# Emieeel/auto_oo

Hardware: AMD Instinct MI355X
Metric: OO-VQE energy+grad evals/sec (formaldimine CAS(4e,3o)/cc-pVDZ); 2e-transform fp64 TFLOP/s vs roofline (higher is better)
Workload: dtype f64; 1 GPU; configs[1] shape: N=43 AOs, n_occ=6, CAS(4e,3o), UCCD n_theta=4, n_kappa=327; one step = one batched call evaluating energy + full gradient of all 256 geometries of the rank (256 synthetic geometries in the job, geometry g on rank g mod n_gpus); value = evaluations/s; in-order calls on one stream; geometries_per_rank=256, batched_calls=1332, calls=in order, parallelism=geometry-sharded x1, one all_gather at the end, dist_world_size=1, devices_visible=1, device_of_rank0=0

## Files before the change

auto_oo_amd/csrc/cas.hip:

```cpp
#include "plan.h"
#include "circuit_small.h"
#include <type_traits>
#include <stdlib.h>

namespace {

constexpr int HALF_WAVES = 8;
constexpr int TRI_REG_R = 3;
constexpr int tiles_depth(int zt) { return zt == 3 ? 4 : 8; }
constexpr int stream_depth(int zt) { return zt == 3 ? 2 : 3; }
constexpr int AUX_PLAIN = 0, AUX_NT = 2;

constexpr int SYM_FULL = 0, SYM_MIRROR = 1, SYM_PACKED = 2;
__device__ __forceinline__ void tri_decode(long t, int N, int& p, int& q)
{
    const double b = 2.0 * N + 1.0;
    int pp = (int)((b - sqrt(b * b - 8.0 * (double)t)) * 0.5);
    pp = pp < 0 ? 0 : (pp > N - 1 ? N - 1 : pp);
    while (pp > 0 && (long)pp * (2 * N - pp + 1) / 2 > t) --pp;
    while (pp < N - 1 && (long)(pp + 1) * (2 * N - pp) / 2 <= t) ++pp;
    p = pp;
    q = pp + (int)(t - (long)pp * (2 * N - pp + 1) / 2);
}

// ... 2241 lines not shown
    double* d1 = lds;
    double* d2 = d1 + (size_t)M * no;
    double* o1 = d2 + (size_t)M * no;
    double* o2 = o1 + (size_t)no * na2;
    double* cube = o2 + (size_t)no * na2;
    double* FIn = cube + na3;
    double* red = FIn + 64;
    for (int idx = tid; idx < M * no; idx += FROW_THREADS) {
        const int x = idx / no, i = idx - x * no;
        d1[idx] = gn[x * M2 + i * M + i];
        d2[idx] = gn[i * M2 + i * M + x];
    }
    for (int idx = tid; idx < no * na2; idx += FROW_THREADS) {
        const int m = idx / na2, vw = idx - m * na2, v = vw / na, w = vw - v * na;
        o1[idx] = gn[m * M2 + (no + v) * M + no + w];
        o2[idx] = gn[(no + w) * M2 + (no + v) * M + m];
    }
    for (int idx = tid; idx < na3; idx += FROW_THREADS) {
        int t = idx;
        const int y = t % na; t /= na;
        const int x = t % na; t /= na;
        cube[idx] = gn[(no + t) * M2 + (no + x) * M + no + y];
    }
    __syncthreads();
    for (int x = tid; x < M; x += FROW_THREADS) {
        double fi = hmo[(size_t)n * M + x];
        for (int i = 0; i < no; ++i) fi += 2.0 * d1[x * no + i] - d2[x * no + i];
        FIn[x] = fi;
    }
    __syncthreads();
    for (int m = tid; m < M; m += FROW_THREADS) {
        double val;
        if (m < no) {
            double fa = 0.0;
            for (int vw = 0; vw < na2; ++vw) fa += gam[vw] * (o1[m * na2 + vw] - 0.5 * o2[m * na2 + vw]);
            val = 2.0 * ((k == 0 ? FIn[m] : 0.0) + fa);
        } else {
            const int v = m - no;
            const double* Gv = Gam + (size_t)v * na3;
            double acc = 0.0;
            for (int w = 0; w < na; ++w) acc += FIn[no + w] * gam[v * na + w];
            for (int idx = 0; idx < na3; ++idx) acc += Gv[idx] * cube[idx];
            val = acc;
        }
        Fcol[((size_t)k * M + m) * N + n] = val;
    }
    double part = 0.0;
    if (n >= no && n < M) {
        const int p = n - no;
        const double* gp = gam + (size_t)p * na;
        const double* Gp = Gam + (size_t)p * na3;
        for (int q = tid; q < na; q += FROW_THREADS) part += FIn[no + q] * gp[q];
        for (int idx = tid; idx < na3; idx += FROW_THREADS) part += 0.5 * cube[idx] * Gp[idx];
    }
    for (int o = 32; o > 0; o >>= 1) part += __shfl_xor(part, o);
    if ((tid & 63) == 0) red[tid >> 6] = part;
    __syncthreads();
    if (tid == 0) Epart[(size_t)k * N + n] = (red[0] + red[1]) + (red[2] + red[3]);
    if (k == 0) {
        if (tid == 0) Cpart[n] = n < no ? hmo[(size_t)n * M + n] + FIn[n] : 0.0;
        if (n >= no && n < M) {
            const int p = n - no;
            for (int q = tid; q < na; q += FROW_THREADS) c1[p * na + q] = FIn[no + q];
            for (int idx = tid; idx < na3; idx += FROW_THREADS) c2[(size_t)p * na3 + idx] = 0.5 * cube[idx];
        }
    }
}

__global__ __launch_bounds__(512)
void cas_final_kernel(const double* __restrict__ Fcol, const double* __restrict__ Epart,
                      const double* __restrict__ Cpart, double nuc, int nrdm, int N, int M,
                      const int32_t* __restrict__ kap_row, const int32_t* __restrict__ kap_col,
                      int n_kappa, double* __restrict__ c0, double* __restrict__ E,
                      double* __restrict__ gvec, double* __restrict__ dE, double* __restrict__ fock,
                      double* __restrict__ gmat, const double* __restrict__ nuc_arr,
                      size_t out_stride)
{
    const int tid = threadIdx.x;
    {
        const size_t gi = blockIdx.x;
        Fcol += gi * (size_t)nrdm * M * N;
        Epart += gi * (size_t)nrdm * N;
        Cpart += gi * (size_t)N;
        c0 += gi * out_stride;
        E += gi * out_stride;
        gvec += gi * out_stride;
        if (dE) dE += gi * out_stride;
        if (fock) fock += gi * (size_t)N * N;
        if (gmat) gmat += gi * (size_t)N * N;
        if (nuc_arr) nuc = nuc_arr[gi];
    }
    for (long base = 0; base < (long)nrdm * n_kappa; base += 4 * 512) {
        int rr[4], cc[4], kk[4];
#pragma unroll
        for (int u = 0; u < 4; ++u) {
            const long idx = base + u * 512 + tid;
            const bool ok = idx < (long)nrdm * n_kappa;
            const long ii = ok ? idx : 0;
            kk[u] = (int)(ii / n_kappa);
            const int t = (int)(ii - (long)kk[u] * n_kappa);
            rr[u] = kap_row[t];
            cc[u] = kap_col[t];
        }
        double frc[4], fcr[4];
#pragma unroll
        for (int u = 0; u < 4; ++u) {
            const double* F = Fcol + (size_t)kk[u] * M * N;
            const int r = rr[u], c = cc[u];
            frc[u] = F[(size_t)(r < M ? r : 0) * N + c] * (r < M ? 1.0 : 0.0);
            fcr[u] = F[(size_t)(c < M ? c : 0) * N + r] * (c < M ? 1.0 : 0.0);
        }
#pragma unroll
        for (int u = 0; u < 4; ++u) {
            const long idx = base + u * 512 + tid;
            if (idx < (long)nrdm * n_kappa) gvec[idx] = 2.0 * (frc[u] - fcr[u]);
        }
    }
    if (fock)
        for (int idx = tid; idx < N * N; idx += 512) {
            const int m = idx / N;
            fock[idx] = m < M ? Fcol[idx] : 0.0;
        }
    if (gmat)
        for (int idx = tid; idx < N * N; idx += 512) {
            const int m = idx / N, n = idx - m * N;
            const double fmn = m < M ? Fcol[(size_t)m * N + n] : 0.0;
            const double fnm = n < M ? Fcol[(size_t)n * N + m] : 0.0;
            gmat[idx] = 2.0 * (fmn - fnm);
        }
    if (tid < nrdm) {
        const int k = tid;
        double acc = 0.0;
        for (int n = 0; n < M; ++n) acc += Epart[(size_t)k * N + n];
        if (k == 0) {
            double core = nuc;
            for (int n = 0; n < M; ++n) core += Cpart[n];
            c0[0] = core;
            E[0] = core + acc;
        } else if (dE) {
            dE[k - 1] = acc;
        }
    }
}

constexpr int TAIL_THREADS = 512;

__host__ __device__ inline bool tail_needed(int x, int y, int z, int no)
{
    const int lo = y < z ? y : z, hi = y < z ? z : y;
    if (lo >= no) return true;
    if (hi < no) return lo == hi || x == lo || x == hi;
    return x >= no || x == lo;
}

#ifdef OOVQE_TAIL_PROBE
constexpr int TAIL_PROBE_WGS = 512, TAIL_PROBE_MARKS = 32;
__device__ long long g_tail_probe[TAIL_PROBE_WGS][TAIL_PROBE_MARKS];
#define TAIL_MARK(i)                                                                              \
    do {                                                                                          \
        __syncthreads();                                                                          \
        if (threadIdx.x == 0 && blockIdx.x < TAIL_PROBE_WGS && (i) < TAIL_PROBE_MARKS)            \
            g_tail_probe[blockIdx.x][i] = wall_clock64();                                         \
    } while (0)
#else
#define TAIL_MARK(i) do {} while (0)
#endif

template <int KS>
__global__ __launch_bounds__(TAIL_THREADS, 2)
void cas_tail_kernel(const double* __restrict__ J, const double* __restrict__ C, const double* __restrict__ Wpre,
                     const double* __restrict__ gamma, const double* __restrict__ Gamma, int nrdm, int N, int no,
                     int na, int NC, double nuc, const double* __restrict__ nuc_arr,
                     const int32_t* __restrict__ kap_row, const int32_t* __restrict__ kap_col, int n_kappa,
                     double* __restrict__ c0, double* __restrict__ E, double* __restrict__ gvec,
                     double* __restrict__ dE, double* __restrict__ c1, double* __restrict__ c2, size_t out_stride)
{
    extern __shared__ double lds[];
    constexpr int NW = TAIL_THREADS / 64;
    constexpr int PW = (4 * KS + NW - 1) / NW;
    constexpr int GR = 2, NG = (PW + GR - 1) / GR;
    constexpr int NTN = (4 * KS + 15) / 16;
    const int M = no + na, M2 = M * M, M3 = M2 * M;
    const int na2 = na * na, na3 = na2 * na, na4 = na2 * na2;
    const int ncol = M * (M + 1) / 2, nty = (ncol + 15) / 16;
    const long tri = (long)N * (N + 1) / 2;
    const int by = blockIdx.x;
    const int tid = threadIdx.x, lane = tid & 63;
    const int wave = __builtin_amdgcn_readfirstlane(tid >> 6);
    const int lq = lane >> 4, lr = lane & 15;
    {
        const size_t gi = by;
        J += gi * nty * tri * 16;
        C += gi * (size_t)N * N;
        Wpre += gi * (size_t)N * N;
        gamma += gi * (size_t)nrdm * na2;
        Gamma += gi * (size_t)nrdm * na4;
        c0 += gi * out_stride;
        E += gi * out_stride;
        gvec += gi * out_stride;
        if (dE) dE += gi * out_stride;
        c1 += gi * out_stride;
        c2 += gi * out_stride;
        if (nuc_arr) nuc = nuc_arr[gi];
    }
    double* Gc = lds;
    double* Cl = Gc + (size_t)N * NC;
    double* hn = Cl + (size_t)N * M;
    double* FIn = hn + (size_t)N * M;
    double* gml = FIn + (size_t)N * M;
    double* Gml = gml + (size_t)nrdm * na2;
    double* Cp = Gml + (size_t)nrdm * na4;
    int* tab = reinterpret_cast<int*>(Cp + N);
    int* wcnt = tab + M3;
    int* krow = wcnt + NW;
    int* kcol = krow + n_kappa;
    double* scr = Cp + N + (M3 + NW + 2 * n_kappa + 1) / 2;
    const int LDP = M * 16 + 8;

    typedef unsigned v2u __attribute__((ext_vector_type(2)));
    const __amdgpu_buffer_rsrc_t csrd = __builtin_amdgcn_make_buffer_rsrc(
        const_cast<double*>(C), 0, (int)((size_t)N * N * sizeof(double)), 0x00020000);
    double cfa[NTN][KS];
#pragma unroll
    for (int nt = 0; nt < NTN; ++nt)
#pragma unroll
        for (int ks = 0; ks < KS; ++ks) {
            const int pp = 4 * ks + lq, n = 16 * nt + lr;
            const v2u v = __builtin_amdgcn_raw_buffer_load_b64(
                csrd, (pp < N && n < N) ? (unsigned)((pp * N + n) * (int)sizeof(double)) : 0x7fffffffu, 0, 0);
            cfa[nt][ks] = __builtin_bit_cast(double, v);
        }
    constexpr bool COLQ_REGS = KS < 12;
    int colq[KS];
#pragma unroll
    for (int ks = 0; ks < KS; ++ks) {
        const int q = 4 * ks + lq < N ? 4 * ks + lq : N - 1;
        colq[ks] = ((q * (2 * N - q + 1) / 2 - q) * 16 + lr) * (int)sizeof(double);
    }
    const int lin0 = (lq * 16 + lr) * (int)sizeof(double);
    auto load_group = [&](double (&bf)[GR][KS], int ty, int g) {
#pragma unroll
        for (int r = 0; r < GR; ++r) {
            const int i = g * GR + r;
            if (i >= PW) continue;
            int wv = wave;
#if defined(__HIP_DEVICE_COMPILE__)
            asm volatile("" : "+s"(wv));
#endif
            const int p = wv + NW * i;
            int lqo = lq;
#if defined(__HIP_DEVICE_COMPILE__)
            asm volatile("" : "+v"(lqo));
#endif
            const __amdgpu_buffer_rsrc_t jsrd = __builtin_amdgcn_make_buffer_rsrc(
                const_cast<double*>(J + (size_t)(ty < nty ? ty : 0) * tri * 16), 0,
                p < N && ty < nty ? (int)(tri * 16 * sizeof(double)) : 0, 0x00020000);
            const int colp = p * 16 * (int)sizeof(double);
            const int rowp = (p * (2 * N - p + 1) / 2 - p) * 16 * (int)sizeof(double) + lin0;
#pragma unroll
            for (int ks = 0; ks < KS; ++ks) {
                const int q = 4 * ks + lqo;
                const int cq = COLQ_REGS ? colq[ks] : (q * (2 * N - 1 - q) / 2 * 16 + lr) * (int)sizeof(double);
                const int off = lq < p - 4 * ks ? cq + colp : rowp + ks * 64 * (int)sizeof(double);
                const v2u v = __builtin_amdgcn_raw_buffer_load_b64(jsrd, (unsigned)off, 0, 0);
                bf[r][ks] = __builtin_bit_cast(double, v);
            }
        }
    };
    double* T3s = scr;
    auto mfma_group = [&](const double (&af)[KS], const double (&bf)[GR][KS], int g) {
#pragma unroll
        for (int r = 0; r < GR; ++r) {
            const int i = g * GR + r;
            if (i >= PW) continue;
            int wv = wave;
#if defined(__HIP_DEVICE_COMPILE__)
            asm volatile("" : "+s"(wv));
#endif
            const int p = wv + NW * i;
            if (p >= 4 * KS) continue;
            d4 acc = d4{0.0, 0.0, 0.0, 0.0};
            if (p < N) {
#pragma unroll
                for (int ks = 0; ks < KS; ++ks) acc = mfma_f64(af[ks], bf[r][ks], acc);
            }
            double* row = T3s + (p * LDP + lq * 16 + lr);
#pragma unroll
            for (int j = 0; j < 4; ++j)
                if (lq + 4 * j < M) row[j * 64] = acc[j];
        }
    };
    double bs[2][GR][KS];
    TAIL_MARK(0);
#pragma unroll
    for (int s0 = 0; s0 < 2; ++s0) load_group(bs[s0], s0 / NG, s0 % NG);

    for (int idx = tid; idx < N * M; idx += TAIL_THREADS) {
        const int q = idx / M, x = idx - q * M;
        Cl[idx] = C[(size_t)q * N + x];
    }
    for (int idx = tid; idx < N * N; idx += TAIL_THREADS) scr[idx] = Wpre[idx];
    for (int idx = tid; idx < nrdm * na2; idx += TAIL_THREADS) gml[idx] = gamma[idx];
    for (int idx = tid; idx < nrdm * na4; idx += TAIL_THREADS) Gml[idx] = Gamma[idx];
    for (int idx = tid; idx < n_kappa; idx += TAIL_THREADS) {
        krow[idx] = kap_row[idx];
        kcol[idx] = kap_col[idx];
    }
    TAIL_MARK(1);
    {
        const int total = M * ncol;
        int base = 0;
        for (int i0 = 0; i0 < total; i0 += TAIL_THREADS) {
            const int i = i0 + tid;
            int x = 0, y = 0, z = 0;
            bool need = false;
            if (i < total) {
                x = i / ncol;
                tri_decode(i - x * ncol, M, y, z);
                need = tail_needed(x, y, z, no);
            }
            const unsigned long long mask = __ballot(need);
            const int below = __popcll(mask & ((1ull << lane) - 1ull));
            if (lane == 0) wcnt[wave] = __popcll(mask);
            __syncthreads();
            int pre = base, all = 0;
            for (int w = 0; w < NW; ++w) {
                const int c = wcnt[w];
                if (w < wave) pre += c;
                all += c;
            }
            if (i < total) {
                const int v = need ? pre + below : -1;
                tab[(x * M + y) * M + z] = v;
                tab[(x * M + z) * M + y] = v;
            }
            __syncthreads();
            base += all;
        }
    }
    TAIL_MARK(2);
    for (int idx = tid; idx < N * M; idx += TAIL_THREADS) {
        const int n = idx / M, x = idx - n * M;
        double acc = 0.0;
        for (int q = 0; q < N; ++q) acc += scr[(size_t)n * N + q] * Cl[q * M + x];
        hn[idx] = acc;
    }
    __syncthreads();
    TAIL_MARK(3);

    {
        const int ntn = (N + 15) / 16;
        auto tail_tile = [&](auto par, int ty) {
            constexpr int P = decltype(par)::value;
            double af[KS];
            int lqv = lq;
#if defined(__HIP_DEVICE_COMPILE__)
            asm volatile("" : "+v"(lqv));
#endif
#pragma unroll
            for (int ks = 0; ks < KS; ++ks) {
                const int q = 4 * ks + lqv;
                const double c = Cl[(q < N ? q : N - 1) * M + (lr < M ? lr : 0)];
                af[ks] = (q < N && lr < M) ? c : 0.0;
            }
#pragma unroll
            for (int g = 0; g < NG; ++g) {
                mfma_group(af, bs[(P + g) & 1], g);
                __builtin_amdgcn_sched_barrier(0);
                load_group(bs[(P + g) & 1], ty + (g + 2) / NG, (g + 2) % NG);
                __builtin_amdgcn_sched_barrier(0);
                if (g == 0) TAIL_MARK(ty < 3 ? 4 + 3 * ty : 31);
            }
            __syncthreads();
            TAIL_MARK(ty < 3 ? 5 + 3 * ty : 31);
            const int yz = 16 * ty + lr;
            int off = 0;
            if (yz < ncol) {
                int y, z;
                tri_decode(yz, M, y, z);
                off = y * M + z;
            }
#pragma unroll
            for (int nt = 0; nt < NTN; ++nt) {
                if (nt >= ntn) continue;
                const int t0 = nt * M;
                for (int tile = t0 + (wave - t0 % NW + NW) % NW; tile < t0 + M; tile += NW) {
                    const int x = tile - t0;
                    double tf[KS];
#pragma unroll
                    for (int ks = 0; ks < KS; ++ks) tf[ks] = T3s[(size_t)(4 * ks + lq) * LDP + x * 16 + lr];
                    d4 acc = d4{0.0, 0.0, 0.0, 0.0};
#pragma unroll
                    for (int ks = 0; ks < KS; ++ks) acc = mfma_f64(cfa[nt][ks], tf[ks], acc);
                    const int ci = yz < ncol ? tab[x * M2 + off] : -1;
                    if (ci >= 0) {
#pragma unroll
                        for (int j = 0; j < 4; ++j) {
                            const int n = 16 * nt + lq + 4 * j;
                            if (n < N) Gc[(size_t)n * NC + ci] = acc[j];
                        }
                    }
                }
            }
            __syncthreads();
            TAIL_MARK(ty < 3 ? 6 + 3 * ty : 31);
        };
        for (int ty = 0; ty < nty; ty += 2) {
            tail_tile(std::integral_constant<int, 0>{}, ty);
            if (ty + 1 < nty) tail_tile(std::integral_constant<int, NG & 1>{}, ty + 1);
        }
    }

#define TAIL_G(n, a, b, c) Gc[(size_t)(n) * NC + tab[((a) * M + (b)) * M + (c)]]
    for (int idx = tid; idx < N * M; idx += TAIL_THREADS) {
        const int n = idx / M, x = idx - n * M;
        double fi = hn[idx];
        for (int i = 0; i < no; ++i) fi += 2.0 * TAIL_G(n, x, i, i) - TAIL_G(n, i, i, x);
        FIn[idx] = fi;
    }
    TAIL_MARK(13);
    double* Fl = scr;
    double* El = Fl + (size_t)nrdm * M * N;
    double* Ga = El + (size_t)nrdm * N;
    double* Dc = Ga + (size_t)N * na3;
    for (int idx = tid; idx < N * na3; idx += TAIL_THREADS) {
        const int n = idx / na3, r = idx - n * na3;
        const int w = r / na2, x = (r / na) % na, y = r % na;
        Ga[idx] = TAIL_G(n, no + w, no + x, no + y);
    }
    for (int idx = tid; idx < N * no * na2; idx += TAIL_THREADS) {
        const int n = idx / (no * na2), r = idx - n * (no * na2);
        const int m = r / na2, v = (r / na) % na, w = r % na;
        const int V = no + v, W = no + w;
        Dc[idx] = TAIL_G(n, m, V, W) - 0.5 * TAIL_G(n, W, V, m);
    }
    __syncthreads();
    TAIL_MARK(14);
    for (int n = tid; n < N; n += TAIL_THREADS) Cp[n] = n < no ? hn[n * M + n] + FIn[n * M + n] : 0.0;
    for (int idx = tid; idx < na * (na + na3); idx += TAIL_THREADS) {
        const int pl = idx / (na + na3), r0 = idx - pl * (na + na3);
        const int n = no + pl;
        if (r0 < na) {
            c1[pl * na + r0] = FIn[n * M + no + r0];
        } else {
            int t = r0 - na;
            const int i3 = t;
            const int s = t % na; t /= na;
            const int r = t % na; t /= na;
            const int q = t;
            c2[(size_t)pl * na3 + i3] = 0.5 * TAIL_G(n, no + q, no + r, no + s);
        }
    }
    TAIL_MARK(15);
    const int ncore = N * nrdm * no;
    for (int idx = tid; idx < N * nrdm * M; idx += TAIL_THREADS) {
        int n, k, m;
        if (idx < ncore) {
            n = idx / (nrdm * no);
            const int r0 = idx - n * (nrdm * no);
            k = r0 / no;
            m = r0 - k * no;
        } else {
            const int j = idx - ncore;
            n = j / (nrdm * na);
            const int r0 = j - n * (nrdm * na);
            k = r0 / na;
            m = no + r0 - k * na;
        }
        const double* FIv = FIn + (size_t)n * M;
        const double* gam = gml + (size_t)k * na2;
        double val;
        if (m < no) {
            const double* Dm = Dc + ((size_t)n * no + m) * na2;
            double fa = 0.0;
            for (int v = 0; v < na; ++v)
                for (int w = 0; w < na; ++w) fa += gam[v * na + w] * Dm[v * na + w];
            val = 2.0 * ((k == 0 ? FIv[m] : 0.0) + fa);
        } else {
            const int v = m - no;
            const double* Gv = Gml + (size_t)k * na4 + (size_t)v * na3;
            double acc = 0.0;
            for (int w = 0; w < na; ++w) acc += FIv[no + w] * gam[v * na + w];
            for (int w = 0; w < na; ++w)
                for (int x = 0; x < na; ++x)
                    for (int y = 0; y < na; ++y)
                        acc += Gv[(w * na + x) * na + y] * Ga[(size_t)n * na3 + (w * na + x) * na + y];
            val = acc;
        }
        Fl[((size_t)k * M + m) * N + n] = val;
    }
    TAIL_MARK(16);
    for (int idx = tid; idx < N * nrdm; idx += TAIL_THREADS) {
        const int n = idx / nrdm, k = idx - n * nrdm;
        double acc = 0.0;
        if (n >= no && n < M) {
            const int p = n - no;
            const double* FIv = FIn + (size_t)n * M;
            const double* gam = gml + (size_t)k * na2 + (size_t)p * na;
            const double* Gpq = Gml + (size_t)k * na4 + (size_t)p * na3;
            for (int q = 0; q < na; ++q) acc += FIv[no + q] * gam[q];
            for (int q = 0; q < na; ++q)
                for (int r = 0; r < na; ++r)
                    for (int s2 = 0; s2 < na; ++s2)
                        acc += 0.5 * Ga[(size_t)n * na3 + (q * na + r) * na + s2] * Gpq[(q * na + r) * na + s2];
        }
        El[(size_t)k * N + n] = acc;
    }
#undef TAIL_G
    __syncthreads();
    TAIL_MARK(17);

    for (int idx = tid; idx < nrdm * n_kappa; idx += TAIL_THREADS) {
        const int k = idx / n_kappa, t = idx - k * n_kappa;
        const int r = krow[t], c = kcol[t];
        const double* F = Fl + (size_t)k * M * N;
        const double frc = F[(size_t)(r < M ? r : 0) * N + c] * (r < M ? 1.0 : 0.0);
        const double fcr = F[(size_t)(c < M ? c : 0) * N + r] * (c < M ? 1.0 : 0.0);
        gvec[idx] = 2.0 * (frc - fcr);
    }
    if (tid < nrdm) {
        const int k = tid;
        double acc = 0.0;
        for (int n = 0; n < M; ++n) acc += El[(size_t)k * N + n];
        if (k == 0) {
            double core = nuc;
            for (int n = 0; n < M; ++n) core += Cp[n];
            c0[0] = core;
            E[0] = core + acc;
        } else if (dE) {
            dE[k - 1] = acc;
        }
    }
    TAIL_MARK(18);
}

}

#ifdef OOVQE_TAIL_PROBE
extern "C" int oovqe_tail_probe_read(long long* out, int n)
{
    const size_t bytes = sizeof(long long) * (size_t)(n < TAIL_PROBE_WGS * TAIL_PROBE_MARKS ? n : TAIL_PROBE_WGS * TAIL_PROBE_MARKS);
    return hipMemcpyFromSymbol(out, HIP_SYMBOL(g_tail_probe), bytes) == hipSuccess ? 0 : 1;
}
#endif

#define OOVQE_STAGE1_DISPATCH(v, LAUNCH, ...)                                                     \
    switch ((v).kch) {                                                                            \
    case 4: LAUNCH(4, 1, 2, ##__VA_ARGS__); break;                                                \
    case 8: LAUNCH(8, 2, 5, ##__VA_ARGS__); break;                                                \
    case 11: LAUNCH(11, 3, 8, ##__VA_ARGS__); break;                                              \
    default: LAUNCH(12, 3, 10, ##__VA_ARGS__); break;                                             \
    }
#define OOVQE_KS_DISPATCH(v, LAUNCH)                                                              \
    switch ((v).ks) {                                                                             \
    case 4: LAUNCH(4); break;                                                                     \
    case 8: LAUNCH(8); break;                                                                     \
    default: LAUNCH(12); break;                                                                   \
    }

static int stage1_variant(int N, Stage1Variant* v)
{
    static const Stage1Variant rows[] = {{4, 1, 2, 4}, {8, 2, 5, 8}, {11, 3, 8, 12}, {12, 3, 10, 12}};
    for (const Stage1Variant& r : rows)
        if (N >= 1 && (N + 3) / 4 <= r.kch) {
            *v = r;
            return 0;
        }
    oovqe_set_error("cas_eval: no stage-1 kernel variant for N=%d", N);
    return OOVQE_ERR_ARG;
}

static size_t half_lds_bytes(int N, int M)
{
    const int ZT = (M + 15) / 16, nrb = (N + 15) / 16, LDM = 16 * (ZT | 1);
    return (((size_t)nrb * 16 * LDM + 511) / 512) * 512 * sizeof(double);
}
static size_t half_lds_bytes_rs(int N, int M) { return half_lds_bytes(N, M) + (size_t)HALF_WAVES * 16 * 17 * sizeof(double); }

static int stage1_half(int N, int M, int sym, bool rs, bool tiles, Stage1* s)
{
    memset(s, 0, sizeof(*s));
    OOVQE_REQUIRE(N >= 1 && M >= 1 && M <= N, "cas_half_transform: bad N=%d M=%d", N, M);
    const int ZT = (M + 15) / 16, nrb = (N + 15) / 16, ksteps = (N + 3) / 4;
    OOVQE_REQUIRE(ZT <= 3, "cas_half_transform: n_occ+ncas = %d > 48 not supported", M);
    OOVQE_REQUIRE(half_lds_bytes(N, M) <= 160 * 1024, "cas_half_transform: N=%d M=%d needs %zu B of LDS", N, M,
                  half_lds_bytes(N, M));
    s->zt = ZT;
    s->sym = sym;
    if (nrb <= 3) {
        s->kernel = S1_HALF;
        if (int rc = stage1_variant(N, &s->v)) return rc;
        snprintf(s->name, sizeof(s->name), "half_transform_kernel<%d,%d,%d>%s", ZT, s->v.kch, s->v.nrb,
                 sym ? " (slabs p <= q)" : "");
        return 0;
    }
    int waste = 1 << 30;
    for (int k = 16; k >= 10; --k) {
        const int w = (ksteps + k - 1) / k * k - ksteps;
        if (w < waste) { waste = w; s->skch = k; }
    }
    s->rs = rs && half_lds_bytes_rs(N, M) <= 160 * 1024;
    if (tiles && s->rs && sym == SYM_MIRROR) {
        s->kernel = S1_TILES;
        snprintf(s->name, sizeof(s->name), "half_tiles_kernel<%d,%d>", ZT, tiles_depth(ZT));
    } else {
        s->kernel = S1_STREAM;
        snprintf(s->name, sizeof(s->name), "half_stream_kernel<%d,%d,%d,%s>", ZT, s->skch, stream_depth(ZT), s->rs ? "true" : "false");
    }
    return 0;
}

static int half_transform_batched(const double* g_ao, const double* C, int N, int M, double* T2, int batch,
                                  oovqe_stream_t stream, const Stage1& s, double* Vk_tri = nullptr,
                                  const double* g_tiles = nullptr)
{
    OOVQE_REQUIRE(g_ao && C && T2, "cas_half_transform: null pointer");
    OOVQE_REQUIRE(!Vk_tri || (s.sym == SYM_MIRROR && N <= 48),
                  "cas_half_transform: the quarter-transformed output needs p<->q symmetric integrals and N <= 48");
    OOVQE_REQUIRE(batch >= 1 && batch <= 65535, "cas_half_transform: batch=%d", batch);
    OOVQE_REQUIRE(s.kernel != S1_TILES || g_tiles, "cas_half_transform: no tile-packed integrals");
    hipStream_t st = (hipStream_t)stream;
    const int ZT = s.zt, sym = s.sym;
    const int nrb = (N + 15) / 16;
    const long nslabs = sym == SYM_FULL ? (long)N * N : (long)N * (N + 1) / 2;
    const long want = (nslabs + HALF_WAVES - 1) / HALF_WAVES;
    oovqe_note_stage1("%s", s.name);
    oovqe_profile_mark_start(st);
    if (s.kernel == S1_HALF) {
#define OOVQE_LAUNCH_HALF(KC_, NS_, NPC_, Z)                                                      \
    do {                                                                                          \
        const unsigned wpg = 4u;                                                \
        hipLaunchKernelGGL((half_transform_kernel<Z, KC_, NS_>),                                  \
                           dim3((unsigned)((nslabs + wpg - 1) / wpg), batch), dim3(wpg * 64),     \
                           0, st, g_ao, C, T2, N, M, nslabs, sym, Vk_tri);                        \
    } while (0)
        if (ZT == 1) OOVQE_STAGE1_DISPATCH(s.v, OOVQE_LAUNCH_HALF, 1)
        else if (ZT == 2) OOVQE_STAGE1_DISPATCH(s.v, OOVQE_LAUNCH_HALF, 2)
        else OOVQE_STAGE1_DISPATCH(s.v, OOVQE_LAUNCH_HALF, 3)
#undef OOVQE_LAUNCH_HALF
    } else if (s.kernel == S1_TILES) {
        const long slab_doubles = (long)nrb * (nrb + 1) / 2 * 256;
        const size_t lds_rs = half_lds_bytes_rs(N, M);
#define OOVQE_LAUNCH_TILES(Z, D_, A_)                                                             \
    do {                                                                                          \
        const void* fn = (const void*)half_tiles_kernel<Z, D_, A_>;                               \
        int rc_ = oovqe_ensure_dynamic_lds(fn, 160 * 1024);                                       \
        if (rc_) return rc_;                                                                      \
        long per = (long)oovqe_cu_count() / batch;               \
        if (per < 1) per = 1;                                                                     \
        if (per > want) per = want;                                                               \
        hipLaunchKernelGGL((half_tiles_kernel<Z, D_, A_>), dim3((unsigned)per, batch),            \
                           dim3(HALF_WAVES * 64), lds_rs, st, g_tiles, C, T2, N, M, nrb, nslabs,  \
                           nslabs * slab_doubles);                                                \
    } while (0)
        if (ZT == 1) OOVQE_LAUNCH_TILES(1, tiles_depth(1), AUX_NT);
        else if (ZT == 3) OOVQE_LAUNCH_TILES(3, tiles_depth(3), AUX_NT);
        else OOVQE_LAUNCH_TILES(2, tiles_depth(2), AUX_NT);
#undef OOVQE_LAUNCH_TILES
    } else {
        const int snkc = ((N + 3) / 4 + s.skch - 1) / s.skch;
#define OOVQE_LAUNCH_STREAM(Z, KC_, D_)                                                           \
    do {                                                                                          \
        if (s.rs) OOVQE_LAUNCH_STREAM_RS(Z, KC_, D_, true, half_lds_bytes_rs(N, M));              \
        else OOVQE_LAUNCH_STREAM_RS(Z, KC_, D_, false, half_lds_bytes(N, M));                     \
    } while (0)
#define OOVQE_LAUNCH_STREAM_RS(Z, KC_, D_, RS_, lds_bytes_)                                       \
    do {                                                                                          \
        const void* fn = (const void*)half_stream_kernel<Z, KC_, D_, RS_>;                        \
        const size_t lds_bytes = lds_bytes_;                                                      \
        if (int rc_ = oovqe_ensure_dynamic_lds(fn, 160 * 1024)) return rc_;                       \
        const int occ = oovqe_blocks_per_cu(fn, HALF_WAVES * 64, lds_bytes);                      \
        if (occ < 0) return occ;                                                                  \
        long per = ((long)occ * oovqe_cu_count()) / batch;                                        \
        if (per < 1) per = 1;                                                                     \
        if (per > want) per = want;                                                               \
        hipLaunchKernelGGL((half_stream_kernel<Z, KC_, D_, RS_>), dim3((unsigned)per, batch),     \
                           dim3(HALF_WAVES * 64), lds_bytes, st, g_ao, C, T2, N, M, nrb, snkc,    \
                           nslabs, sym);                                                          \
    } while (0)
#define OOVQE_DISPATCH_STREAM(Z, D_)                                                              \
    do {                                                                                          \
        switch (s.skch) {                                                                         \
        case 10: OOVQE_LAUNCH_STREAM(Z, 10, D_); break;                                           \
        case 11: OOVQE_LAUNCH_STREAM(Z, 11, D_); break;                                           \
        case 12: OOVQE_LAUNCH_STREAM(Z, 12, D_); break;                                           \
        case 13: OOVQE_LAUNCH_STREAM(Z, 13, D_); break;                                           \
// ... 4 lines not shown
    } while (0)
        if (ZT == 1) OOVQE_DISPATCH_STREAM(1, stream_depth(1));
        else if (ZT == 2) OOVQE_DISPATCH_STREAM(2, stream_depth(2));
        else OOVQE_DISPATCH_STREAM(3, stream_depth(3));
#undef OOVQE_DISPATCH_STREAM
#undef OOVQE_LAUNCH_STREAM
#undef OOVQE_LAUNCH_STREAM_RS
    }
    oovqe_profile_mark_stop(st);
    OOVQE_CHECK_LAUNCH(s.kernel == S1_TILES ? "cas_half_transform/tiles" : "cas_half_transform");
    return 0;
}

extern "C" int oovqe_cas_half_transform(const double* g_ao, const double* C, int N, int M, double* T2,
                                        oovqe_stream_t stream)
{
    Stage1 s;
    if (int rc = stage1_half(N, M, SYM_FULL, false, false, &s)) return rc;
    return half_transform_batched(g_ao, C, N, M, T2, 1, stream, s);
}

extern "C" int oovqe_eri_symmetry_flags(const double* g_ao, int N, int batch, unsigned* eri_flags,
                                        oovqe_stream_t stream)
{
    OOVQE_REQUIRE(g_ao && eri_flags, "eri_symmetry_flags: null pointer");
    OOVQE_REQUIRE(N >= 1 && N <= 65535 && batch >= 1 && batch <= 65535, "eri_symmetry_flags: N=%d batch=%d",
                  N, batch);
    hipStream_t st = (hipStream_t)stream;
    int* flag = nullptr;
    OOVQE_CHECK_HIP(hipMalloc(&flag, sizeof(int)), "eri_symmetry_flags");
    hipError_t e = hipMemsetAsync(flag, 0, sizeof(int), st);
    if (e == hipSuccess) {
        hipLaunchKernelGGL(eri_symmetry_check_kernel, dim3(N, N, batch), dim3(256), 0, st,
                           reinterpret_cast<const unsigned long long*>(g_ao), N, flag);
        e = hipGetLastError();
    }
    int bad = 3;
    if (e == hipSuccess) e = hipMemcpyAsync(&bad, flag, sizeof(int), hipMemcpyDeviceToHost, st);
    if (e == hipSuccess) e = hipStreamSynchronize(st);
    (void)hipFree(flag);
    OOVQE_CHECK_HIP(e, "eri_symmetry_flags");
    *eri_flags = ((bad & 1) ? 0u : OOVQE_ERI_PQ_SYMMETRIC) | ((bad & 2) ? 0u : OOVQE_ERI_RS_SYMMETRIC);
    return 0;
}

extern "C" int oovqe_eri_ingest(const double* g_ao, int N, int batch, double* packed, unsigned* eri_flags,
                                oovqe_stream_t stream)
{
    OOVQE_REQUIRE(g_ao && eri_flags, "eri_ingest: null pointer");
    OOVQE_REQUIRE(N >= 1 && N <= 4096 && batch >= 1 && batch <= 65535, "eri_ingest: N=%d batch=%d", N, batch);
    hipStream_t st = (hipStream_t)stream;
    if (N > 48) {
        for (int gi = 0; gi < batch; ++gi) {
            int rc = oovqe_eri_symmetry_flags(g_ao + (size_t)gi * N * N * N * N, N, 1, eri_flags + gi, stream);
            if (rc) return rc;
        }
        return packed ? oovqe_eri_pack(g_ao, N, batch, packed, stream) : 0;
    }
    int* flag = nullptr;
    OOVQE_CHECK_HIP(hipMalloc(&flag, sizeof(int) * (size_t)batch), "eri_ingest");
    hipError_t e = hipMemsetAsync(flag, 0, sizeof(int) * (size_t)batch, st);
    if (e == hipSuccess) {
        hipLaunchKernelGGL(eri_ingest_kernel, dim3((unsigned)(N * (N + 1) / 2), batch), dim3(256), 0, st,
                           reinterpret_cast<const unsigned long long*>(g_ao), packed, N, eri_slab_pitch(N), flag);
        e = hipGetLastError();
    }
    int* bad = (int*)malloc(sizeof(int) * (size_t)batch);
    if (!bad) e = hipErrorOutOfMemory;
    if (e == hipSuccess) e = hipMemcpyAsync(bad, flag, sizeof(int) * (size_t)batch, hipMemcpyDeviceToHost, st);
    if (e == hipSuccess) e = hipStreamSynchronize(st);
    (void)hipFree(flag);
    if (e == hipSuccess)
        for (int gi = 0; gi < batch; ++gi)
            eri_flags[gi] = ((bad[gi] & 1) ? 0u : OOVQE_ERI_PQ_SYMMETRIC) | ((bad[gi] & 2) ? 0u : OOVQE_ERI_RS_SYMMETRIC);
    free(bad);
    OOVQE_CHECK_HIP(e, "eri_ingest");
    return 0;
}

static int sym_q_contract_batched(const double* J, const double* C, double* T3, int N, int M, int batch,
                                  hipStream_t st)
{
    OOVQE_REQUIRE(M >= 1 && M <= 16 && N >= 1 && N <= 48, "sym_q_contract: N=%d M=%d", N, M);
    Stage1Variant v;
    if (int rc = stage1_variant(N, &v)) return rc;
    const unsigned threads = (unsigned)((M * M + 15) / 16 * 64);
    oovqe_profile_mark_start_l(st, LABEL_Q_TO_X);
#define OOVQE_LAUNCH_Q(KS_) \
    hipLaunchKernelGGL(sym_q_contract_kernel<KS_>, dim3(N, batch), dim3(threads), 0, st, J, C, T3, N, M)
    OOVQE_KS_DISPATCH(v, OOVQE_LAUNCH_Q)
#undef OOVQE_LAUNCH_Q
    oovqe_profile_mark_stop(st);
    OOVQE_CHECK_LAUNCH("cas_eval/sym_q_contract");
    return 0;
}

static int sym_gm_batched(const double* J, const double* C, double* Gm, int N, int M, int batch,
                          hipStream_t st, const oovqe_circuit_job_t* cj, bool packed)
{
    OOVQE_REQUIRE(M >= 1 && M <= 16 && N >= 1 && N <= 48, "sym_gm: N=%d M=%d", N, M);
    Stage1Variant v;
    if (int rc = stage1_variant(N, &v)) return rc;
    size_t lds_bytes = (size_t)4 * v.ks * (M * 16 + 8) * sizeof(double);
    if (cj && cj->lds_bytes > lds_bytes) lds_bytes = cj->lds_bytes;
    const unsigned nty = (unsigned)(((packed ? M * (M + 1) / 2 : M * M) + 15) / 16);
    oovqe_circuit_job_t job;
    memset(&job, 0, sizeof(job));
    if (cj) job = *cj;
    const unsigned nx = nty + (cj ? 1 : 0);
    const bool xcd_grid = batch > 1 && oovqe_opt(OOVQE_OPT_GM_PLAIN_GRID) == 0;
    const dim3 grid = xcd_grid ? dim3(nx * (unsigned)((batch + 7) / 8 * 8)) : dim3(nx, batch);
#define OOVQE_LAUNCH_GM2(KS_, WPE_)                                                               \
    do {                                                                                          \
        if (int rc_ = oovqe_ensure_dynamic_lds((const void*)sym_gm_kernel<KS_, WPE_>, lds_bytes)) return rc_; \
        hipLaunchKernelGGL((sym_gm_kernel<KS_, WPE_>), grid, dim3(SMALL_THREADS), lds_bytes, st,  \
                           J, C, Gm, N, M, packed ? 1 : 0, job, cj ? 1 : 0, batch);               \
    } while (0)
    const bool multi_round = ((long)nx * batch > (long)oovqe_cu_count() || oovqe_opt(OOVQE_OPT_GM_TWO_PER_CU)) &&
                             2 * lds_bytes <= 160 * 1024 && oovqe_opt(OOVQE_OPT_GM_ONE_PER_CU) == 0;
#define OOVQE_LAUNCH_GM(KS_)                                                                      \
    do {                                                                                          \
        if (multi_round) OOVQE_LAUNCH_GM2(KS_, 4);                                                \
        else OOVQE_LAUNCH_GM2(KS_, 2);                                                            \
    } while (0)
    oovqe_profile_mark_start_l(st, LABEL_P_TO_N);
    OOVQE_KS_DISPATCH(v, OOVQE_LAUNCH_GM)
    oovqe_profile_mark_stop(st);
#undef OOVQE_LAUNCH_GM
#undef OOVQE_LAUNCH_GM2
    OOVQE_CHECK_LAUNCH("cas_eval/sym_gm");
    return 0;
}

static int tail_depth(int N, const Stage1Variant& v) { return N >= 41 && N <= 44 ? 11 : v.ks; }
#define OOVQE_TAIL_DISPATCH(ks, LAUNCH)                                                           \
    switch (ks) {                                                                                 \
    case 4: LAUNCH(4); break;                                                                     \
    case 8: LAUNCH(8); break;                                                                     \
    case 11: LAUNCH(11); break;                                                                   \
    default: LAUNCH(12); break;                                                                   \
    }

static size_t tail_lds_bytes(int N, int no, int na, int nrdm, int n_kappa, int* NC)
{
    const int M = no + na, M3 = M * M * M;
    Stage1Variant v;
    if (N > 48 || M > 16 || stage1_variant(N, &v)) return 0;
    int nc = 0;
    for (int x = 0; x < M; ++x)
        for (int y = 0; y < M; ++y)
            for (int z = y; z < M; ++z) nc += tail_needed(x, y, z, no) ? 1 : 0;
    *NC = nc;
    const size_t na2 = (size_t)na * na, na4 = na2 * na2;
    size_t scr = (size_t)N * N;
    const size_t t3 = (size_t)4 * tail_depth(N, v) * (M * 16 + 8);
    const size_t fe = (size_t)nrdm * M * N + (size_t)nrdm * N +
                      (size_t)N * na * na * na + (size_t)N * no * na2;
    if (t3 > scr) scr = t3;
    if (fe > scr) scr = fe;
    const size_t doubles = (size_t)N * nc + 3 * (size_t)N * M + (size_t)nrdm * (na2 + na4) + N +
                           ((size_t)M3 + TAIL_THREADS / 64 + 2 * (size_t)n_kappa + 1) / 2 + scr;
    const size_t bytes = doubles * sizeof(double);
    return bytes <= 160 * 1024 ? bytes : 0;
}

static int cas_tail_batched(const CasEvalArgs& a, const EvalPlan& p, const double* J, const double* Wpre, hipStream_t st)
{
    Stage1Variant v;
    if (int rc = stage1_variant(a.N, &v)) return rc;
#define OOVQE_LAUNCH_TAIL(KS_)                                                                    \
    do {                                                                                          \
        if (int rc_ = oovqe_ensure_dynamic_lds((const void*)cas_tail_kernel<KS_>, p.tail_lds)) return rc_; \
        hipLaunchKernelGGL((cas_tail_kernel<KS_>), dim3(a.batch), dim3(TAIL_THREADS), p.tail_lds, st, J, a.C, Wpre, \
                           a.gamma, a.Gamma, a.nrdm, a.N, a.n_occ, a.ncas, p.tail_nc, a.nuc, a.nuc_arr, a.kap_row, \
                           a.kap_col, a.n_kappa, a.out.c0, a.out.E, a.out.gvec, a.out.dE, a.out.c1, a.out.c2,       \
                           a.out_stride);                                                         \
    } while (0)
    oovqe_profile_mark_start_l(st, LABEL_P_TO_N);
    OOVQE_TAIL_DISPATCH(tail_depth(a.N, v), OOVQE_LAUNCH_TAIL)
    oovqe_profile_mark_stop(st);
#undef OOVQE_LAUNCH_TAIL
    OOVQE_CHECK_LAUNCH("cas_eval/tail");
    return 0;
}

static bool fused_plan(int N, int M, int batch, int n_cu, long chunks_opt, FusedPlan* fp)
{
    if (M > 16 || N > 48 || N < 1) return false;
    const long m2 = (long)M * M, m3 = m2 * M;
    if (chunks_opt <= 0 && (long)batch * N * N < 48L * n_cu) return false;
    long target = n_cu / batch;
    long nchunk0 = chunks_opt > 0 ? chunks_opt : target / N;
    if (nchunk0 < 1) nchunk0 = 1;
    const long cap = (2L * N * m2 - m3) / (m3 + N);
    if (cap < 1) return false;
    if (nchunk0 > cap) nchunk0 = cap;
    int qc = N, nchunk = 1;
    if (nchunk0 > 1) {
        qc = 4 * (int)((N + 4 * nchunk0 - 1) / (4 * nchunk0));
        nchunk = (N + qc - 1) / qc;
    }
    const int QR = (qc + 3) & ~3, CR = (nchunk - 1) * qc + QR;
    int ldb = (int)((m2 + 15) / 16 * 16);
    if (ldb % 32 == 0) ldb += 16;
    const size_t fixed = ((size_t)CR * 16 + 64 + 8) * sizeof(double);
    const size_t block = (size_t)QR * ldb * sizeof(double);
    const size_t task_stage = (size_t)m3 * sizeof(double);
    const long Tg = (long)nchunk * N;
    long wpg = target < 1 ? 1 : target;
    if (wpg > Tg) wpg = Tg;
    const size_t lds_cap = 160 * 1024;
    if (fixed + 2 * block + task_stage > lds_cap) return false;
    const long max_tasks = (long)((lds_cap - fixed - 2 * block) / task_stage);
    if ((Tg + wpg - 1) / wpg > max_tasks) wpg = (Tg + max_tasks - 1) / max_tasks;
    const long ntask = (Tg + wpg - 1) / wpg;
    long nbuf = (long)((lds_cap - fixed - (size_t)ntask * task_stage) / block);
    if (nbuf > 3) nbuf = 3;
    fp->nchunk = nchunk;
    fp->qc = qc;
    fp->nbuf = (int)nbuf;
    fp->ldb = ldb;
    fp->wpg = (int)wpg;
    fp->lds_bytes = fixed + (size_t)nbuf * block + (size_t)ntask * task_stage;
    return true;
}

static int half_transform_fused_batched(const double* g_ao, const double* C, int N, int M, double* T3,
                                        double* Cdup, const FusedPlan& fp, const Stage1& s, int batch, hipStream_t st)
{
#define OOVQE_LAUNCH_FUSED(KC_, NS_, NPC_)                                                        \
    do {                                                                                          \
        if (int rc_lds = oovqe_ensure_dynamic_lds((const void*)half_transform_fused_kernel<KC_, NS_>, 160 * 1024)) return rc_lds; \
        hipLaunchKernelGGL((half_transform_fused_kernel<KC_, NS_>), dim3(fp.wpg, batch),          \
                           dim3(HALF_WAVES * 64), fp.lds_bytes, st, g_ao, C, T3, Cdup, N, M,      \
                           fp.nchunk, fp.qc, fp.nbuf, fp.ldb);                                    \
    } while (0)
    oovqe_note_stage1("%s", s.name);
    oovqe_profile_mark_start(st);
    OOVQE_STAGE1_DISPATCH(s.v, OOVQE_LAUNCH_FUSED)
    oovqe_profile_mark_stop(st);
#undef OOVQE_LAUNCH_FUSED
    OOVQE_CHECK_LAUNCH("cas_eval/half_transform_fused");
    return 0;
}

static unsigned eri_slab_packed_elems(int N) { return eri_slab_pitch(N); }

extern "C" int64_t oovqe_eri_packed_size(int N)
{
    if (N < 1) return 0;
    if (N > 48) {
        const int64_t nst = (N + 15) / 16;
        return (int64_t)N * (N + 1) / 2 * (nst * (nst + 1) / 2) * 256;
    }
    return (int64_t)N * (N + 1) / 2 * eri_slab_packed_elems(N);
}

extern "C" int oovqe_eri_pack(const double* g_ao, int N, int batch, double* packed, oovqe_stream_t stream)
{
    OOVQE_REQUIRE(g_ao && packed, "eri_pack: null pointer");
    OOVQE_REQUIRE(N >= 1 && N <= 4096 && batch >= 1 && batch <= 65535, "eri_pack: N=%d batch=%d", N, batch);
    if (N > 48) {
        hipLaunchKernelGGL(eri_tiles_pack_kernel, dim3((unsigned)((long)N * (N + 1) / 2), batch), dim3(256), 0,
                           (hipStream_t)stream, g_ao, packed, N, (N + 15) / 16);
        OOVQE_CHECK_LAUNCH("eri_pack/tiles");
        return 0;
    }
    hipLaunchKernelGGL(eri_pack_kernel, dim3((unsigned)(N * (N + 1) / 2), batch), dim3(256), 0,
                       (hipStream_t)stream, g_ao, packed, N, eri_slab_packed_elems(N));
    OOVQE_CHECK_LAUNCH("eri_pack");
    return 0;
}

static int half_tri_batched(const double* g_ao, const double* C, int N, int M, double* J, int batch,
                            hipStream_t st, const Stage1& s)
{
    const int tiled = s.tiled;
    const bool packed_src = s.kernel == S1_TRI_REG;
    OOVQE_REQUIRE(!packed_src || tiled == 2, "cas_eval: packed integrals need both symmetry flags");
    OOVQE_REQUIRE(M >= 1 && M <= 16 && N >= M && N <= 48, "cas_eval: half_tri N=%d M=%d", N, M);
    const long tri = (long)N * (N + 1) / 2;
    const long n_cu = oovqe_cu_count();
    const long w_max = (tri + HALF_WAVES - 1) / HALF_WAVES;
    long W = n_cu / batch;
    if (W < 1) W = 1;
    if (W > w_max) W = w_max;
    if (oovqe_opt(OOVQE_OPT_TRI_PLAIN_W) == 0) {
        auto cost = [&](long w) {
            return ((long)batch * w + n_cu - 1) / n_cu * ((tri + w * HALF_WAVES - 1) / (w * HALF_WAVES) + 3);
        };
        long best = cost(W);
        for (long w = 1; w <= 16 && w <= w_max; ++w)
            if (cost(w) < best) { best = cost(w); W = w; }
    }
    const long n_rounds = (tri + W * HALF_WAVES - 1) / (W * HALF_WAVES);
    const size_t round_bytes = (size_t)HALF_WAVES * M * M * sizeof(double);
    const size_t fixed_bytes = (64 + 128) * sizeof(double);
    if (packed_src) {
        const int npc = s.v.npc;
        OOVQE_REQUIRE((size_t)npc * 1024 >= eri_slab_packed_elems(N) * sizeof(double),
                      "cas_eval: half_tri_reg slab of N=%d exceeds %d KB", N, npc);
        constexpr int R = TRI_REG_R;
        const size_t slot_bytes = (size_t)HALF_WAVES * npc * 1024;
        long ph = (long)((160 * 1024 - fixed_bytes - slot_bytes) / round_bytes) / R * R;
        OOVQE_REQUIRE(ph >= R, "cas_eval: half_tri_reg staging does not fit LDS (M=%d)", M);
        const long nr_up = (n_rounds + R - 1) / R * R;
        if (ph > nr_up) ph = nr_up;
        const size_t lds_reg = fixed_bytes + slot_bytes + (size_t)ph * round_bytes;
#define OOVQE_LAUNCH_TRI_REG(KC_, NS_, NPC_)                                                      \
    do {                                                                                          \
        if (int rc_ = oovqe_ensure_dynamic_lds((const void*)half_tri_reg_kernel<KC_, NS_, NPC_, R>, 160 * 1024)) return rc_; \
        hipLaunchKernelGGL((half_tri_reg_kernel<KC_, NS_, NPC_, R>), dim3((unsigned)W, batch),    \
                           dim3(HALF_WAVES * 64), lds_reg, st, g_ao, C, J, N, M, (int)ph);        \
// ... 750 lines not shown
```

Before: 588,100 evals/s.

## Restructure CAS tail transform: scatter half-transformed tiles then one batched C back-transform

Instead of transforming each tile pair back through C immediately (with syncs per tile and a T3 scratch buffer), the tail kernel now scatters first-stage MFMA results straight into a padded Gc buffer using a precomputed packed index table. It then runs a single second-stage pass over column tiles with C fragments loaded just before it. This removes per-tile __syncthreads and the tri_decode/table lookups, hoists the af fragment load out of the tile loop, and uses an odd-multiple pitch to reduce LDS bank conflicts. The cost is a different LDS layout sized 4*KS*pitch, extra zero-fill of padding, and a later cfa load that cannot overlap the stream.

```diff
diff --git a/auto_oo_amd/csrc/cas.hip b/auto_oo_amd/csrc/cas.hip
--- a/auto_oo_amd/csrc/cas.hip
+++ b/auto_oo_amd/csrc/cas.hip
@@ -2417,6 +2417,7 @@
     if (hi < no) return lo == hi || x == lo || x == hi;
     return x >= no || x == lo;
 }
+__host__ __device__ inline int tail_pitch(int NC) { return 16 * (((NC + 15) / 16) | 1); }
 
 #ifdef OOVQE_TAIL_PROBE
 constexpr int TAIL_PROBE_WGS = 512, TAIL_PROBE_MARKS = 32;
@@ -2468,8 +2469,9 @@
         c2 += gi * out_stride;
         if (nuc_arr) nuc = nuc_arr[gi];
     }
+    const int LDG = tail_pitch(NC), nct = (NC + 15) / 16;
     double* Gc = lds;
-    double* Cl = Gc + (size_t)N * NC;
+    double* Cl = Gc + (size_t)4 * KS * LDG;
     double* hn = Cl + (size_t)N * M;
     double* FIn = hn + (size_t)N * M;
     double* gml = FIn + (size_t)N * M;
@@ -2480,21 +2482,9 @@
     int* krow = wcnt + NW;
     int* kcol = krow + n_kappa;
     double* scr = Cp + N + (M3 + NW + 2 * n_kappa + 1) / 2;
-    const int LDP = M * 16 + 8;
+    int* tabp = reinterpret_cast<int*>(scr + (size_t)N * N);
 
     typedef unsigned v2u __attribute__((ext_vector_type(2)));
-    const __amdgpu_buffer_rsrc_t csrd = __builtin_amdgcn_make_buffer_rsrc(
-        const_cast<double*>(C), 0, (int)((size_t)N * N * sizeof(double)), 0x00020000);
-    double cfa[NTN][KS];
-#pragma unroll
-    for (int nt = 0; nt < NTN; ++nt)
-#pragma unroll
-        for (int ks = 0; ks < KS; ++ks) {
-            const int pp = 4 * ks + lq, n = 16 * nt + lr;
-            const v2u v = __builtin_amdgcn_raw_buffer_load_b64(
-                csrd, (pp < N && n < N) ? (unsigned)((pp * N + n) * (int)sizeof(double)) : 0x7fffffffu, 0, 0);
-            cfa[nt][ks] = __builtin_bit_cast(double, v);
-        }
     constexpr bool COLQ_REGS = KS < 12;
     int colq[KS];
 #pragma unroll
@@ -2532,8 +2522,7 @@
             }
         }
     };
-    double* T3s = scr;
-    auto mfma_group = [&](const double (&af)[KS], const double (&bf)[GR][KS], int g) {
+    auto mfma_group = [&](const double (&af)[KS], const double (&bf)[GR][KS], const int (&tj)[4], int g) {
 #pragma unroll
         for (int r = 0; r < GR; ++r) {
             const int i = g * GR + r;
@@ -2549,10 +2538,10 @@
 #pragma unroll
                 for (int ks = 0; ks < KS; ++ks) acc = mfma_f64(af[ks], bf[r][ks], acc);
             }
-            double* row = T3s + (p * LDP + lq * 16 + lr);
+            double* row = Gc + p * LDG;
 #pragma unroll
             for (int j = 0; j < 4; ++j)
-                if (lq + 4 * j < M) row[j * 64] = acc[j];
+                if (tj[j] >= 0) row[tj[j]] = acc[j];
         }
     };
     double bs[2][GR][KS];
@@ -2570,6 +2559,10 @@
     for (int idx = tid; idx < n_kappa; idx += TAIL_THREADS) {
         krow[idx] = kap_row[idx];
         kcol[idx] = kap_col[idx];
+    }
+    for (int idx = tid; idx < 4 * KS * (LDG - NC); idx += TAIL_THREADS) {
+        const int p = idx / (LDG - NC);
+        Gc[p * LDG + NC + (idx - p * (LDG - NC))] = 0.0;
     }
     TAIL_MARK(1);
     {
@@ -2598,6 +2591,7 @@
                 const int v = need ? pre + below : -1;
                 tab[(x * M + y) * M + z] = v;
                 tab[(x * M + z) * M + y] = v;
+                tabp[i] = v;
             }
             __syncthreads();
             base += all;
@@ -2614,61 +2608,29 @@
     TAIL_MARK(3);
 
     {
-        const int ntn = (N + 15) / 16;
+        double af[KS];
+#pragma unroll
+        for (int ks = 0; ks < KS; ++ks) {
+            const int q = 4 * ks + lq;
+            const double c = Cl[(q < N ? q : N - 1) * M + (lr < M ? lr : 0)];
+            af[ks] = (q < N && lr < M) ? c : 0.0;
+        }
         auto tail_tile = [&](auto par, int ty) {
             constexpr int P = decltype(par)::value;
-            double af[KS];
-            int lqv = lq;
-#if defined(__HIP_DEVICE_COMPILE__)
-            asm volatile("" : "+v"(lqv));
-#endif
-#pragma unroll
-            for (int ks = 0; ks < KS; ++ks) {
-                const int q = 4 * ks + lqv;
-                const double c = Cl[(q < N ? q : N - 1) * M + (lr < M ? lr : 0)];
-                af[ks] = (q < N && lr < M) ? c : 0.0;
+            const int yz = 16 * ty + lr;
+            int tj[4];
+#pragma unroll
+            for (int j = 0; j < 4; ++j) {
+                const int x = lq + 4 * j;
+                tj[j] = (x < M && yz < ncol) ? tabp[x * ncol + yz] : -1;
             }
 #pragma unroll
             for (int g = 0; g < NG; ++g) {
-                mfma_group(af, bs[(P + g) & 1], g);
+                mfma_group(af, bs[(P + g) & 1], tj, g);
                 __builtin_amdgcn_sched_barrier(0);
                 load_group(bs[(P + g) & 1], ty + (g + 2) / NG, (g + 2) % NG);
                 __builtin_amdgcn_sched_barrier(0);
-                if (g == 0) TAIL_MARK(ty < 3 ? 4 + 3 * ty : 31);
-            }
-            __syncthreads();
-            TAIL_MARK(ty < 3 ? 5 + 3 * ty : 31);
-            const int yz = 16 * ty + lr;
-            int off = 0;
-            if (yz < ncol) {
-                int y, z;
-                tri_decode(yz, M, y, z);
-                off = y * M + z;
-            }
-#pragma unroll
-            for (int nt = 0; nt < NTN; ++nt) {
-                if (nt >= ntn) continue;
-                const int t0 = nt * M;
-                for (int tile = t0 + (wave - t0 % NW + NW) % NW; tile < t0 + M; tile += NW) {
-                    const int x = tile - t0;
-                    double tf[KS];
-#pragma unroll
-                    for (int ks = 0; ks < KS; ++ks) tf[ks] = T3s[(size_t)(4 * ks + lq) * LDP + x * 16 + lr];
-                    d4 acc = d4{0.0, 0.0, 0.0, 0.0};
-#pragma unroll
-                    for (int ks = 0; ks < KS; ++ks) acc = mfma_f64(cfa[nt][ks], tf[ks], acc);
-                    const int ci = yz < ncol ? tab[x * M2 + off] : -1;
-                    if (ci >= 0) {
-#pragma unroll
-                        for (int j = 0; j < 4; ++j) {
-                            const int n = 16 * nt + lq + 4 * j;
-                            if (n < N) Gc[(size_t)n * NC + ci] = acc[j];
-                        }
-                    }
-                }
-            }
-            __syncthreads();
-            TAIL_MARK(ty < 3 ? 6 + 3 * ty : 31);
+            }
         };
         for (int ty = 0; ty < nty; ty += 2) {
             tail_tile(std::integral_constant<int, 0>{}, ty);
@@ -2676,14 +2638,52 @@
         }
     }
 
-#define TAIL_G(n, a, b, c) Gc[(size_t)(n) * NC + tab[((a) * M + (b)) * M + (c)]]
+    {
+        const __amdgpu_buffer_rsrc_t csrd = __builtin_amdgcn_make_buffer_rsrc(
+            const_cast<double*>(C), 0, (int)((size_t)N * N * sizeof(double)), 0x00020000);
+        double cfa[NTN][KS];
+#pragma unroll
+        for (int nt = 0; nt < NTN; ++nt)
+#pragma unroll
+            for (int ks = 0; ks < KS; ++ks) {
+                const int pp = 4 * ks + lq, n = 16 * nt + lr;
+                const v2u v = __builtin_amdgcn_raw_buffer_load_b64(
+                    csrd, (pp < N && n < N) ? (unsigned)((pp * N + n) * (int)sizeof(double)) : 0x7fffffffu, 0, 0);
+                cfa[nt][ks] = __builtin_bit_cast(double, v);
+            }
+        __syncthreads();
+        TAIL_MARK(4);
+        const int ntn = (N + 15) / 16;
+        for (int ct = wave; ct < nct; ct += NW) {
+            double* col = Gc + (16 * ct + lr);
+            double tf[KS];
+#pragma unroll
+            for (int ks = 0; ks < KS; ++ks) tf[ks] = col[(4 * ks + lq) * LDG];
+#pragma unroll
+            for (int nt = 0; nt < NTN; ++nt) {
+                if (nt >= ntn) continue;
+                d4 acc = d4{0.0, 0.0, 0.0, 0.0};
+#pragma unroll
+                for (int ks = 0; ks < KS; ++ks) acc = mfma_f64(cfa[nt][ks], tf[ks], acc);
+#pragma unroll
+                for (int j = 0; j < 4; ++j) {
+                    const int n = 16 * nt + lq + 4 * j;
+                    if (n < N) col[n * LDG] = acc[j];
+                }
+            }
+        }
+        __syncthreads();
+        TAIL_MARK(5);
+    }
+
+#define TAIL_G(n, a, b, c) Gc[(n) * LDG + tab[((a) * M + (b)) * M + (c)]]
     for (int idx = tid; idx < N * M; idx += TAIL_THREADS) {
         const int n = idx / M, x = idx - n * M;
         double fi = hn[idx];
         for (int i = 0; i < no; ++i) fi += 2.0 * TAIL_G(n, x, i, i) - TAIL_G(n, i, i, x);
         FIn[idx] = fi;
     }
-    TAIL_MARK(13);
+    TAIL_MARK(6);
     double* Fl = scr;
     double* El = Fl + (size_t)nrdm * M * N;
     double* Ga = El + (size_t)nrdm * N;
@@ -2700,7 +2700,7 @@
         Dc[idx] = TAIL_G(n, m, V, W) - 0.5 * TAIL_G(n, W, V, m);
     }
     __syncthreads();
-    TAIL_MARK(14);
+    TAIL_MARK(7);
     for (int n = tid; n < N; n += TAIL_THREADS) Cp[n] = n < no ? hn[n * M + n] + FIn[n * M + n] : 0.0;
     for (int idx = tid; idx < na * (na + na3); idx += TAIL_THREADS) {
         const int pl = idx / (na + na3), r0 = idx - pl * (na + na3);
@@ -2716,7 +2716,7 @@
             c2[(size_t)pl * na3 + i3] = 0.5 * TAIL_G(n, no + q, no + r, no + s);
         }
     }
-    TAIL_MARK(15);
+    TAIL_MARK(8);
     const int ncore = N * nrdm * no;
     for (int idx = tid; idx < N * nrdm * M; idx += TAIL_THREADS) {
         int n, k, m;
@@ -2754,7 +2754,7 @@
         }
         Fl[((size_t)k * M + m) * N + n] = val;
     }
-    TAIL_MARK(16);
+    TAIL_MARK(9);
     for (int idx = tid; idx < N * nrdm; idx += TAIL_THREADS) {
         const int n = idx / nrdm, k = idx - n * nrdm;
         double acc = 0.0;
@@ -2773,7 +2773,7 @@
     }
 #undef TAIL_G
     __syncthreads();
-    TAIL_MARK(17);
+    TAIL_MARK(10);
 
     for (int idx = tid; idx < nrdm * n_kappa; idx += TAIL_THREADS) {
         const int k = idx / n_kappa, t = idx - k * n_kappa;
@@ -2796,7 +2796,7 @@
             dE[k - 1] = acc;
         }
     }
-    TAIL_MARK(18);
+    TAIL_MARK(11);
 }
 
 }
@@ -3107,13 +3107,12 @@
             for (int z = y; z < M; ++z) nc += tail_needed(x, y, z, no) ? 1 : 0;
     *NC = nc;
     const size_t na2 = (size_t)na * na, na4 = na2 * na2;
-    size_t scr = (size_t)N * N;
-    const size_t t3 = (size_t)4 * tail_depth(N, v) * (M * 16 + 8);
+    size_t scr = (size_t)N * N + ((size_t)M * (M * (M + 1) / 2) + 1) / 2;
+    const size_t gc = (size_t)4 * tail_depth(N, v) * tail_pitch(nc);
     const size_t fe = (size_t)nrdm * M * N + (size_t)nrdm * N +
                       (size_t)N * na * na * na + (size_t)N * no * na2;
-    if (t3 > scr) scr = t3;
     if (fe > scr) scr = fe;
-    const size_t doubles = (size_t)N * nc + 3 * (size_t)N * M + (size_t)nrdm * (na2 + na4) + N +
+    const size_t doubles = gc + 3 * (size_t)N * M + (size_t)nrdm * (na2 + na4) + N +
                            ((size_t)M3 + TAIL_THREADS / 64 + 2 * (size_t)n_kappa + 1) / 2 + scr;
     const size_t bytes = doubles * sizeof(double);
     return bytes <= 160 * 1024 ? bytes : 0;
```

New measurement: 605,000 evals/s (median of 6 runs). +2.9%, better.
